# yoshihikoueno/DNNCancerAnnotator

Measured on AMD Instinct MI355X. Metric: MRI slices/sec (fwd+bwd) unet 512x512 bs=8, higher is better.
Workload: dtype f32; 1 GPU; configs/unet.yaml train step (fwd + weighted BCE + bwd + Adam), batch 8 x 512x512x1 per GPU, f32, random-init weights; global_batch=8, parallelism=dp1, kernels=tuned, communicator=False

## Files before the change

### dnncancerannotator_amd/csrc/debug_tools.hip

```cpp
#include "fast.h"
#include "kernels.h"
#include "model.h"
#include <vector>

using namespace dnnca;

typedef float dbg_f32x4 __attribute__((ext_vector_type(4)));
template <int MODE, int NCH>
__global__ __launch_bounds__(512) void k_mfma_rate(float* out, int iters) {
    __shared__ float lds[16384];
    for (int i = threadIdx.x; i < 16384; i += 512) lds[i] = (float)(i & 7) * 0.125f;
    __syncthreads();
    const int lane = threadIdx.x & 63, wave = threadIdx.x >> 6;
    dbg_f32x4 acc[NCH];
    for (int c = 0; c < NCH; ++c) acc[c] = dbg_f32x4{0.f, 0.f, 0.f, 0.f};
    float a = 1.0f + lane * 0.001f, b = 0.5f;
    const int base = wave * 1024 + (lane & 15) * 12 + (lane >> 4);
    for (int it = 0; it < iters; ++it) {
#pragma unroll
        for (int k = 0; k < 16; ++k)
#pragma unroll
            for (int c = 0; c < NCH; ++c) {
                float av = MODE >= 1 ? lds[base + c * 200 + 4 * k + (it & 1) * 64] : a;
                float bv = MODE == 2 ? lds[8192 + base + 4 * k + (it & 1) * 64] : b;
// ... 41 lines not shown
int dnnca_debug_bn_table(void* model, double* abs_sum, unsigned* ticket_sum, int* allocated) {
    MODEL(model);
    *abs_sum = 0.0;
    *ticket_sum = 0u;
    *allocated = M->bn_tab != nullptr;
    if (!M->bn_tab) return DNNCA_OK;
    HIP_TRY(hipStreamSynchronize(M->stream));
    std::vector<double> h(Model::kBnTab + 32);
    HIP_TRY(hipMemcpy(h.data(), M->bn_tab, h.size() * 8, hipMemcpyDeviceToHost));
    for (int i = 0; i < Model::kBnTab; ++i) *abs_sum += h[i] < 0 ? -h[i] : h[i];
    const unsigned* t = reinterpret_cast<const unsigned*>(h.data() + Model::kBnTab);
    for (int i = 0; i < 64; ++i) *ticket_sum += t[i];
    return DNNCA_OK;
}

int dnnca_debug_tcf_dgrads(void* model, int batch, float* dskip, size_t n_skip, float* dtcin, size_t n_tcin) {
    MODEL(model);
    for (size_t i = M->ops.size(); i-- > 1;) {
        const Op& o = M->ops[i];
        const Op& tc = M->ops[i - 1];
        if (o.type != OP_CONV || !o.inB.d.C || o.inA.d.C != 3 || o.inB.d.C != 3 || o.out.d.C != 3) continue;
        if (tc.type != OP_TCONV || tc.inA.d.C != 6 || tc.out.d.p != o.inA.d.p) continue;
        const size_t ns = (size_t)batch * o.out.d.H * o.out.d.W * 3, nt = (size_t)batch * tc.inA.d.H * tc.inA.d.W * 6;
        if (ns != n_skip || nt != n_tcin || !o.inB.g.p || !tc.inA.g.p) { set_error("dnnca_debug_tcf_dgrads: sizes %zu / %zu expected", ns, nt); return DNNCA_EINVAL; }
        HIP_TRY(hipStreamSynchronize(M->stream));
        HIP_TRY(hipMemcpy(dskip, o.inB.g.p, ns * 4, hipMemcpyDeviceToHost));
        HIP_TRY(hipMemcpy(dtcin, tc.inA.g.p, nt * 4, hipMemcpyDeviceToHost));
        return DNNCA_OK;
    }
    set_error("dnnca_debug_tcf_dgrads: no two-source 3-channel conv behind a 6 -> 3 transposed conv");
    return DNNCA_EINVAL;
}

int dnnca_debug_join(void* model, int what, int B, int H, int W, int C, int ps, int c0, int grid, int generic, const float* in0,
                     const float* in1, float* io0, float* io1, const float* coef, double* sums, int acc0, int acc1) {
    MODEL(model);
    if (what < 0 || what > 2 || B < 1 || H < 1 || W < 1 || C < 1 || c0 < 0 || c0 + C > ps || !in0 || !in1 || !io0 || (what == 2 && !io1) ||
        (what == 1 && !coef) || (generic && what == 1)) { set_error("dnnca_debug_join: bad arguments"); return DNNCA_EINVAL; }
    const size_t n = (size_t)B * H * W * ps;
    float* dev = nullptr;
    const size_t n4 = (n + 3) / 4 * 4;
    double* dsum = nullptr;
    unsigned* ticket = nullptr;
    float* dcoef = nullptr;
    const unsigned rows = (unsigned)(grid > 0 ? grid : 0) + (unsigned)((C + 255) / 256);
    const size_t part = std::max(join_part_doubles(C), (size_t)rows * C);
    hipStream_t s = M->stream;
    int rc = DNNCA_OK;
    auto body = [&]() -> int {
        HIP_TRY(hipMalloc(&dev, 4 * n4 * 4));
        HIP_TRY(hipMalloc(&dsum, (2 * (size_t)C + part) * 8));
        HIP_TRY(hipMalloc(&ticket, 16));
        HIP_TRY(hipMalloc(&dcoef, 2 * (size_t)C * 4));
        HIP_TRY(hipMemsetAsync(ticket, 0, 16, s));
        HIP_TRY(hipMemsetAsync(dsum, 0xff, (2 * (size_t)C + part) * 8, s));
        HIP_TRY(hipMemcpyAsync(dev, in0, n * 4, hipMemcpyHostToDevice, s));
        HIP_TRY(hipMemcpyAsync(dev + n4, in1, n * 4, hipMemcpyHostToDevice, s));
        HIP_TRY(hipMemcpyAsync(dev + 2 * n4, io0, n * 4, hipMemcpyHostToDevice, s));
        if (io1) HIP_TRY(hipMemcpyAsync(dev + 3 * n4, io1, n * 4, hipMemcpyHostToDevice, s));
        if (coef) HIP_TRY(hipMemcpyAsync(dcoef, coef, 2 * (size_t)C * 4, hipMemcpyHostToDevice, s));
        View v[4];
        for (int k = 0; k < 4; ++k) { v[k].p = dev + k * n4 + c0; v[k].H = H; v[k].W = W; v[k].C = C; v[k].ps = ps; }
        if (what == 0) {
            if (generic) g_join_fwd(s, B, v[0], v[1], v[2]);
            else join_fwd(s, B, v[0], v[1], v[2], sums ? dsum : nullptr, dsum + 2 * C, ticket, grid);
        } else if (what == 1) {
// ... 26 lines not shown
```

### dnncancerannotator_amd/csrc/fz_dev.h

```cpp
#pragma once
#include <hip/hip_runtime.h>

namespace dnnca {
namespace fz {

typedef float f32x4 __attribute__((ext_vector_type(4)));

constexpr int cdiv(int a, int b) { return (a + b - 1) / b; }
constexpr int up4(int a) { return (a + 3) / 4 * 4; }

template <int C, int G, int RG, int ROWS, int HALO>
struct Tile {
    static constexpr int LEAD = (4 - (HALO * C) % 4) % 4;
    static constexpr int LS = RG * G * C;
    static constexpr int LS4 = LS / 4;
    static_assert(LS % 4 == 0, "tile rows must be whole float4's");
    static constexpr int N = up4(LEAD + (ROWS + 2) * LS + 20 * G * C + 16);
    static constexpr int N4 = N / 4;
};

__device__ __forceinline__ void lds_barrier() { asm volatile("s_waitcnt lgkmcnt(0)\n\ts_barrier" ::: "memory"); }
__device__ __forceinline__ float act(float v, float alpha) { return alpha < 0.f ? v : (v > 0.f ? v : alpha * v); }


template <int C, int G, int RG, int ROWS, int HALO, int WPX, int LSF, int NT>
struct Stager {
    static constexpr int LEAD = (4 - (HALO * C) % 4) % 4;
    static constexpr int W4 = (LEAD + WPX * C + 3) / 4;
    static constexpr int LS4 = LSF / 4;
    static_assert(W4 <= LS4 && LSF % 4 == 0, "tile row narrower than the staged width");
    static constexpr int NPF = cdiv(ROWS * W4, NT);
    float4 pre[NPF];
    unsigned ok;
    __device__ __forceinline__ void issue(const float* __restrict__ src, int b, int y0, int x0, int H, int W, int tid) {
        const int rowlen4 = W * C / 4;
        const int f40 = ((x0 - HALO) * C - LEAD) / 4;
        const float4* base = reinterpret_cast<const float4*>(src) + (size_t)b * H * rowlen4;
        const int last = H * rowlen4 - 1;
        ok = 0;
#pragma unroll
        for (int k = 0; k < NPF; ++k) {
            const int idx = tid + k * NT;
            const int r = idx / W4, c4 = idx - r * W4;
            const int gy = y0 - HALO + r, g4 = f40 + c4;
            ok |= (idx < ROWS * W4 && (unsigned)gy < (unsigned)H && (unsigned)g4 < (unsigned)rowlen4) ? (1u << k) : 0u;
            pre[k] = base[min(max(gy * rowlen4 + g4, 0), last)];
        }
    }
    __device__ __forceinline__ void commit(float* lds, int tid) const {
#pragma unroll
        for (int k = 0; k < NPF; ++k) {
            const int idx = tid + k * NT;
            const int r = idx / W4, c4 = idx - r * W4;
            if (idx < ROWS * W4) reinterpret_cast<float4*>(lds)[r * LS4 + c4] = (ok >> k) & 1u ? pre[k] : make_float4(0.f, 0.f, 0.f, 0.f);
        }
    }
};

template <int C, int G, int RG, int ROWS, int HALO, int TW, int TH, int NT>
__device__ __forceinline__ void store_interior(const float* lds, float* __restrict__ dst, int b, int y0, int x0, int H, int W, int tid) {
    using TL = Tile<C, G, RG, ROWS, HALO>;
    constexpr int R4 = TW * C / 4;
    constexpr int OFF = TL::LEAD + HALO * C;
    static_assert(OFF % 4 == 0 && (TW * C) % 4 == 0, "unaligned tile interior");
    float* base = dst + ((size_t)b * H + y0) * W * C + (size_t)x0 * C;
    for (int idx = tid; idx < TH * R4; idx += NT) {
        const int r = idx / R4, c4 = idx - r * R4;
        const float4 v = *reinterpret_cast<const float4*>(lds + (HALO + r) * TL::LS + OFF + 4 * c4);
        *reinterpret_cast<float4*>(base + (size_t)r * W * C + 4 * c4) = v;
    }
}

template <int C, int G, int RG, int OROWS, int OW, int LEAD, int NT>
__device__ __forceinline__ void zero_ring(float* t, unsigned edge, int tid) {
    constexpr int LS = RG * G * C;
    if (edge & 1u) for (int i = tid; i < OW * C; i += NT) t[LEAD + i] = 0.f;
    if (edge & 2u) for (int i = tid; i < OW * C; i += NT) t[LEAD + (OROWS - 1) * LS + i] = 0.f;
    if (edge & 4u) for (int i = tid; i < OROWS * C; i += NT) t[LEAD + (i / C) * LS + (i % C)] = 0.f;
    if (edge & 8u) for (int i = tid; i < OROWS * C; i += NT) t[LEAD + (i / C) * LS + (OW - 1) * C + (i % C)] = 0.f;
}

template <int C, int NSRC, int CO, int RG, int OROWS, int ILEAD, int ISTRIDE, int OLEAD, int NW, int MPR>
struct Conv3 {
    static constexpr int G = 12 / CO, GC = G * C, WR = (G + 2) * C, SR = (WR + 3) / 4, KS = NSRC * 3 * SR, ILS = RG * GC;
    static constexpr int NMT = MPR ? OROWS * MPR : cdiv(OROWS * RG, 16), CH = cdiv(NMT, NW);
    static_assert(MPR == 0 || (NW % MPR == 0 && NMT % NW == 0), "row-aligned M-tiles must divide evenly over the waves");
    static constexpr int CSTEP = MPR ? (NW / MPR) * RG * GC : NW * 16 * GC;
// ... 71 lines not shown
```

### dnncancerannotator_amd/csrc/kernels_fused_bwd.hip

```cpp
#include <stdio.h>
#include <stdlib.h>
#include <string.h>
#include <type_traits>

#include "fast.h"
#include "fz_dev.h"
#include "kernels.h"

namespace dnnca {
namespace fzb {

using namespace fz;

template <int C, int CO, int RG, int OROWS, int ILEAD, int OLEAD, int NW, int MPR>
struct DConv3 {
    static constexpr int G = 12 / CO, GC = G * C, WR = (G + 2) * C, SR = (WR + 3) / 4, KS = 3 * SR, ILS = RG * GC;
    static constexpr int NMT = MPR ? OROWS * MPR : cdiv(OROWS * RG, 16), CH = cdiv(NMT, NW);
    static_assert(MPR == 0 || (NW % MPR == 0 && NMT % NW == 0), "row-aligned M-tiles must divide evenly over the waves");
    static constexpr int CSTEP = MPR ? RG * GC : NW * 16 * GC;

    static __device__ __forceinline__ void run(const float* in, float* out, const float* breg, const float* msk, float malpha, int wave, int lane) {
        const int m = lane & 15, q = lane >> 4, n = m;
        constexpr bool RAGGED = CH * NW > NMT;
        const bool last_ok = !RAGGED || wave + (CH - 1) * NW < NMT;
// ... 100 lines not shown
    do {                                                                                                              \
        if (lane == 0 && (wave == 0 || wave == NWD) && blockIdx.x < 1024 && (i) < 32) g_fzb_stamps[((KID * 1024 + blockIdx.x) * 2 + (role)) * 32 + (i)] = fzb_now(); \
    } while (0)
#else
#define FZB_STAMP(role, i) do { } while (0)
#endif

struct BArgs {
    const float* dz1;
    const float* y1;
    const float* dpool;
    const unsigned char* pidx;
    float pf_alpha;
    const float* y0;
    const float* xa;
    const float* xb;
    const float* bm1;
    const float* bm0;
    float* dxb;
    int mask0;
    float alpha0;
    float* slabs1;
    float* slabs0[2];
    const float* tc_in;
    float* tc_din;
    const float* tc_w;
    float* tc_slabs;
    int tc_mask;
    float tc_alpha;
    int B, H, W, tiles_x, tiles_y;
    int dbg;
};

template <bool UP, int CA, int F, int TW, int NT, int ISSUE_DG = 2, int ISSUE_WG = 2>
__global__ __launch_bounds__(NT, 1) void k_fzb(BArgs p) {
    constexpr int TH = 8, NW = NT / 64, NWD = NW / 2, NWW = NW - NWD, NSRC = UP ? 2 : 1, CT = 12;
    constexpr int KID = (UP ? 0 : 2) + (F == 12 ? 1 : 0);
    (void)KID;
    static_assert(!UP || CA == F, "decoder block: both sources of the first conv have F channels");
    constexpr int G = 12 / F, RG = even_up(cdiv(TW + 5, G)), PR = RG * G;
    using TDZ1 = Tile<F, G, RG, TH + 4, 2>;
    using TY0 = Tile<F, G, RG, TH + 2, 1>;
    using TXA = Tile<CA, G, RG, TH + 2, 1>;
    constexpr int CO2 = UP ? 12 : CA, G2 = 12 / CO2, NPASS = UP ? (2 * F) / 12 : 1, RG2I = PR / G2, MPR2 = (TW / G2) / 16, OUT2 = TH * TW * CO2;
    static_assert(PR % G2 == 0 && (TW / G2) % 16 == 0, "second-stage groups must tile the rows");
    using DC1 = DConv3<F, F, RG, TH + 2, TDZ1::LEAD, TY0::LEAD, NWD, 0>;
    using DC0 = DConv3<F, CO2, RG2I, TH, TY0::LEAD, 0, NWD, MPR2>;
    using W1 = WG<F, F, TW>;
    using W0 = WG<CA, F, TW>;
    using SDZ = Stager<F, G, RG, TH + 4, 2, TW + 4, TDZ1::LS, NT>;
    using SY0 = Stager<F, G, RG, TH + 2, 1, TW + 2, TY0::LS, NT>;
    using SXA = Stager<CA, G, RG, TH + 2, 1, TW + 2, TXA::LS, NT>;
    constexpr int LWt = TW / 2, NLP = (TH / 2) * LWt, KA = 2 * F, KS1t = KA / 4, KTt = 4 * F, MBt = cdiv(KTt, 16), ROWF = TW * 12;
    using SLO = Stager<CT, 1, 1, TH / 2, 0, TW / 2, LWt * CT, NT>;
    static_assert(!UP || (LWt % 16 == 0 && KA % 4 == 0), "UP: whole M-tiles per low-resolution row");
    constexpr int PFR = TH / 2 + 2, PFW = TW / 2 + 2, PFLEAD = (4 - F % 4) % 4, PFLS = up4(PFLEAD + PFW * F), PFLI = PFLS / 4, PFN4 = PFR * PFLI;
    constexpr int NPS = UP ? 1 : cdiv(PFN4, NT);
    constexpr int O_DZ1 = 0, O_Y0 = O_DZ1 + TDZ1::N, O_DZ0 = O_Y0 + TY0::N, O_XA = O_DZ0 + TY0::N, O_EXT = O_XA + NSRC * TXA::N;
    constexpr int O_LOW = O_EXT, O_TCW = O_LOW + NLP * CT;
    constexpr int O_PDP = O_EXT, O_PIX = O_PDP + PFN4 * 4;
    constexpr int O_CST = UP ? O_TCW + KTt * CT : O_PIX + PFN4, O_ROW = O_CST + 4;
    constexpr int O_BM1 = O_ROW + NWD * 192, O_BM0 = O_BM1 + DC1::KS * 64, LDSN = O_BM0 + NPASS * DC0::KS * 64;
    constexpr int O_OUT = O_DZ1;
    static_assert(NPASS * OUT2 <= TDZ1::N, "stage-2 output tiles must fit the dz1 tile");
    constexpr int MT1 = W1::MT, MT0 = W0::MT;
    constexpr int ACCF = (MT1 + NSRC * MT0) * 256;
    constexpr int TACCF = UP ? MBt * 256 : 0;
    static_assert(NWW * ACCF + NWD * TACCF <= LDSN, "the final reduction must fit the LDS");
    constexpr int RPW = TH / (NWD / MPR2), LPW = 8 * (RPW / 2);
    static_assert(NWD % MPR2 == 0 && TH % (NWD / MPR2) == 0 && (!UP || (RPW % 2 == 0 && LPW % 16 == 0)), "wave rectangles");
    static_assert(LDSN * 4 <= 160 * 1024, "LDS budget");
    __shared__ float4 lds4[(LDSN + 3) / 4];
    float* lds = reinterpret_cast<float*>(lds4);
    const float* ldsf = lds;
    constexpr int CST1 = O_CST, CST0 = O_CST + 1;

    const int tid = threadIdx.x, lane = tid & 63;
    const int wave = __builtin_amdgcn_readfirstlane(tid >> 6);
    const int ntiles = p.tiles_x * p.tiles_y * p.B;
#ifdef DNNCA_TUNING
    const bool xcd_map = (ntiles & 7) == 0 && (gridDim.x & 7) == 0 && !(p.dbg & 4);
#else
    const bool xcd_map = (ntiles & 7) == 0 && (gridDim.x & 7) == 0;
#endif

    SDZ sdz;
    SY0 sy0;
    SXA sxa[NSRC];
    SDZ sy1;
    SLO slo;
    float4 predp[NPS];
    unsigned preix[NPS];
    auto issue = [&](int b, int x0, int y0) {
        sdz.issue(p.dz1, b, y0, x0, p.H, p.W, tid);
        if constexpr (!UP) {
            sy1.issue(p.y1, b, y0, x0, p.H, p.W, tid);
            const int Hp = p.H >> 1, Wp = p.W >> 1, rowf = Wp * F;
#pragma unroll
            for (int k = 0; k < NPS; ++k) {
                const int id = tid + k * NT;
                const int r = id / PFLI, c4 = id - r * PFLI;
                const int gy = (y0 >> 1) - 1 + r, gf = ((x0 >> 1) - 1) * F - PFLEAD + 4 * c4;
                const bool ok = id < PFN4 && (unsigned)gy < (unsigned)Hp && gf >= 0 && gf < rowf;
                const size_t off = ok ? ((size_t)b * Hp + gy) * rowf + gf : 0;
                predp[k] = *reinterpret_cast<const float4*>(p.dpool + off);
                if (!ok) predp[k] = make_float4(0.f, 0.f, 0.f, 0.f);
                preix[k] = *reinterpret_cast<const unsigned*>(p.pidx + off);
                if (!ok) preix[k] = 0xffffffffu;
            }
        }
        sy0.issue(p.y0, b, y0, x0, p.H, p.W, tid);
        sxa[0].issue(p.xa, b, y0, x0, p.H, p.W, tid);
        if constexpr (UP) {
            sxa[1].issue(p.xb, b, y0, x0, p.H, p.W, tid);
            slo.issue(p.tc_in, b, y0 >> 1, x0 >> 1, p.H >> 1, p.W >> 1, tid);
        }
    };
    auto commit = [&]() {
        if constexpr (!UP) {
#pragma unroll
            for (int k = 0; k < NPS; ++k) {
                const int id = tid + k * NT;
                if (id < PFN4) {
                    reinterpret_cast<float4*>(lds + O_PDP)[id] = predp[k];
                    reinterpret_cast<unsigned*>(lds + O_PIX)[id] = preix[k];
                }
            }
            lds_barrier();
            const unsigned char* ixb = reinterpret_cast<const unsigned char*>(lds + O_PIX);
            const float* pdp = lds + O_PDP;
            static_assert(SDZ::LEAD == 0 && F % 2 == 0 && PFLS % 2 == 0 && (PFLEAD % 2) == 0, "PF transform works on aligned channel pairs");
#pragma unroll
            for (int k = 0; k < SDZ::NPF; ++k) {
                const int idx = tid + k * NT;
                const int r = idx / SDZ::W4, c4 = idx - r * SDZ::W4;
                float g[4] = {sdz.pre[k].x, sdz.pre[k].y, sdz.pre[k].z, sdz.pre[k].w};
                const float yv[4] = {sy1.pre[k].x, sy1.pre[k].y, sy1.pre[k].z, sy1.pre[k].w};
                const int f0 = 4 * c4;
                if (((sdz.ok >> k) & 1u) && f0 < (TW + 4) * F) {
                    const int px0 = f0 / F, ch0 = f0 - px0 * F;
                    const int pr = ((r - 2) >> 1) + 1;
                    const unsigned rowbit = ((unsigned)r & 1u) << 1;
#pragma unroll
                    for (int h = 0; h < 2; ++h) {
                        int ch = ch0 + 2 * h, px = px0;
                        if (ch >= F) { ch -= F; ++px; }
                        const int pc = ((px - 2) >> 1) + 1;
                        const unsigned pos = rowbit | ((unsigned)px & 1u);
                        const int o = pr * PFLS + PFLEAD + pc * F + ch;
                        const float2 dp = *reinterpret_cast<const float2*>(pdp + o);
                        const unsigned ix = *reinterpret_cast<const unsigned short*>(ixb + o);
                        g[2 * h] = (g[2 * h] + ((ix & 0xffu) == pos ? dp.x : 0.f)) * (yv[2 * h] > 0.f ? 1.0f : p.pf_alpha);
                        g[2 * h + 1] = (g[2 * h + 1] + ((ix >> 8) == pos ? dp.y : 0.f)) * (yv[2 * h + 1] > 0.f ? 1.0f : p.pf_alpha);
                    }
                }
                sdz.pre[k] = make_float4(g[0], g[1], g[2], g[3]);
            }
        }
        sdz.commit(lds + O_DZ1, tid);
        sy0.commit(lds + O_Y0, tid);
        sxa[0].commit(lds + O_XA, tid);
        if constexpr (UP) {
            sxa[1].commit(lds + O_XA + TXA::N, tid);
            slo.commit(lds + O_LOW, tid);
        }
    };

    FZB_STAMP(wave >= NWD, 0);
    int tile = blockIdx.x;
    int b = 0, x0 = 0, y0 = 0;
    if (tile < ntiles) {
        decode_tile(tile, ntiles, xcd_map, p.tiles_x, p.tiles_y, TW, TH, b, x0, y0);
        issue(b, x0, y0);
    }
#ifdef DNNCA_TUNING
    if (p.dbg & 8) {
        FZB_STAMP(wave >= NWD, 25);
        asm volatile("s_waitcnt vmcnt(0)" ::: "memory");
        FZB_STAMP(wave >= NWD, 26);
    }
#endif
    constexpr int KSA = DC1::KS + NPASS * DC0::KS, NBR = cdiv(KSA, NW);
    static_assert(O_BM0 == O_BM1 + DC1::KS * 64, "bm1 and bm0 adjacent in LDS");
    float pbm[NBR];
#pragma unroll
    for (int k = 0; k < NBR; ++k) {
        const int s = min(wave + k * NW, KSA - 1);
        pbm[k] = s < DC1::KS ? p.bm1[s * 64 + lane] : p.bm0[(s - DC1::KS) * 64 + lane];
    }
    constexpr int NTW = UP ? cdiv(KTt * CT, NT) : 1;
    float ptw[NTW];
    if constexpr (UP) {
#pragma unroll
        for (int k = 0; k < NTW; ++k) ptw[k] = p.tc_w[min(tid + k * NT, KTt * CT - 1)];
    }
    FZB_STAMP(wave >= NWD, 27);
    for (int i = tid; i < (LDSN + 3) / 4; i += NT) lds4[i] = make_float4(0.f, 0.f, 0.f, 0.f);
    FZB_STAMP(wave >= NWD, 28);
    __syncthreads();
    FZB_STAMP(wave >= NWD, 29);
    if (tid == 0) lds[CST1] = 1.0f;
#pragma unroll
    for (int k = 0; k < NBR; ++k)
        if (wave + k * NW < KSA) lds[O_BM1 + (wave + k * NW) * 64 + lane] = pbm[k];
    if constexpr (UP) {
#pragma unroll
        for (int k = 0; k < NTW; ++k)
            if (tid + k * NT < KTt * CT) lds[O_TCW + tid + k * NT] = ptw[k];
    }
    if (tile >= ntiles) return;

    int cb = b, cx0 = x0, cy0 = y0;
    FZB_STAMP(wave >= NWD, 1);
    commit();
    tile += gridDim.x;
    lds_barrier();
    FZB_STAMP(wave >= NWD, 2);

    auto role = [&](auto tag) {
        constexpr bool DG = decltype(tag)::value;
        const int wv = DG ? wave : wave - NWD;
        f32x4 acc1[1][MT1], acc0[NSRC][MT0], tacc[UP ? MBt : 1];
        W1 w1;
        W0 w0;
        if constexpr (DG) {
#pragma unroll
            for (int t = 0; t < (UP ? MBt : 1); ++t) tacc[t] = f32x4{0.f, 0.f, 0.f, 0.f};
        }
        if constexpr (!DG) {
#pragma unroll
            for (int t = 0; t < MT1; ++t) acc1[0][t] = f32x4{0.f, 0.f, 0.f, 0.f};
#pragma unroll
            for (int s = 0; s < NSRC; ++s)
#pragma unroll
                for (int t = 0; t < MT0; ++t) acc0[s][t] = f32x4{0.f, 0.f, 0.f, 0.f};
            w1.init(lane, TY0::LEAD, TY0::LS, CST1, CST0);
            w0.init(lane, TXA::LEAD, TXA::LS, CST1, CST0);
        }
        int it = 0;
        (void)it;
#pragma unroll 1
        for (;; ++it) {
            const unsigned edge = tile_edge(cx0, cy0, TW, TH, p.H, p.W);
            FZB_STAMP(!DG, it < 3 ? 3 + 8 * it : 99);
            auto prefetch = [&]() {
                decode_tile(tile < ntiles ? tile : tile - (int)gridDim.x, ntiles, xcd_map, p.tiles_x, p.tiles_y, TW, TH, b, x0, y0);
                issue(b, x0, y0);
            };
            constexpr int ISSUE_AT = DG ? ISSUE_DG : ISSUE_WG;
            if constexpr (ISSUE_AT == 1) prefetch();
            __builtin_amdgcn_s_setprio(DG ? 2 : 0);
            if constexpr (DG) {
                float breg[DC1::KS];
                load_breg<DC1::KS>(breg, lds + O_BM1, lane);
                DC1::run(lds + O_DZ1, lds + O_DZ0, breg, p.mask0 ? lds + O_Y0 : nullptr, p.alpha0, wv, lane);
            } else {
#pragma unroll 1
                for (int ty = wv; ty < TH; ty += NWW) {
                    const int xr[1] = {O_Y0 + ty * TY0::LS};
                    w1.template row<1>(acc1, ldsf, xr, O_DZ1 + TDZ1::LEAD + (ty + 2) * TDZ1::LS + 2 * F, CST0, lane);
                }
            }
            FZB_STAMP(!DG, it < 3 ? 4 + 8 * it : 99);
            lds_barrier();
            FZB_STAMP(!DG, it < 3 ? 5 + 8 * it : 99);
            if (edge && !(p.mask0 && p.alpha0 == 0.f)) {
                zero_ring<F, G, RG, TH + 2, TW + 2, TY0::LEAD, NT>(lds + O_DZ0, edge, tid);
                lds_barrier();
            }
            __builtin_amdgcn_s_setprio(0);
            if constexpr (ISSUE_AT == 2) prefetch();
            if constexpr (DG) {
#pragma unroll
                for (int ps = 0; ps < NPASS; ++ps) {
                    float breg[DC0::KS];
                    load_breg<DC0::KS>(breg, lds + O_BM0 + ps * DC0::KS * 64, lane);
                    DC0::run(lds + O_DZ0, lds + O_OUT + ps * OUT2, breg, nullptr, 0.f, wv, lane);
                }
                __builtin_amdgcn_wave_barrier();
                const int r0 = (wv / MPR2) * RPW, cbk = wv % MPR2;
                if constexpr (UP) {
                    float* base = p.dxb + ((size_t)cb * p.H + cy0 + r0) * p.W * F + (size_t)(cx0 + cbk * 16) * F;
                    if constexpr (NPASS == 2) {
                        static_assert(F == 12, "two passes: 12 channels per pass");
                        if (lane < 48) {
#pragma unroll
                            for (int rr = 0; rr < RPW; ++rr)
                                *reinterpret_cast<float4*>(base + (size_t)rr * p.W * F + 4 * lane) =
                                    *reinterpret_cast<const float4*>(lds + O_OUT + OUT2 + (r0 + rr) * ROWF + cbk * 192 + 4 * lane);
                        }
                    } else {
                        static_assert(F == 6, "one pass: [up | skip] of 6 channels each");
                        if (lane < 48) {
                            const int px = (2 * lane) / F, ch = 2 * lane - px * F;
#pragma unroll
                            for (int rr = 0; rr < RPW; ++rr)
                                *reinterpret_cast<float2*>(base + (size_t)rr * p.W * F + 2 * lane) =
                                    *reinterpret_cast<const float2*>(lds + O_OUT + (r0 + rr) * ROWF + (cbk * 16 + px) * 12 + F + ch);
                        }
                    }
                    const int m16 = lane & 15, q = lane >> 4;
                    const int lr0 = r0 / 2, lc0 = cbk * 8;
                    int koff[KS1t];
#pragma unroll
                    for (int kk = 0; kk < KS1t; ++kk) {
                        const int k = 4 * kk + q, e = k / F;
                        koff[kk] = e * 12 + (k - e * F);
                    }
                    const int woff = m16 < CT ? O_TCW + q * CT + m16 : CST0, wstep = m16 < CT ? 4 * CT : 0;
                    float* orow = lds + O_ROW + wv * 192;
#pragma unroll
// ... 52 lines not shown
#pragma unroll
                        for (int t = 0; t < MBt; ++t) tav[i][t] = ldsf[offT[t] + (valT[t] ? sd : 0)];
                    }
                    __builtin_amdgcn_sched_barrier(0);
#pragma unroll
                    for (int i = 0; i < KST; ++i)
#pragma unroll
                        for (int t = 0; t < MBt; ++t) tacc[t] = __builtin_amdgcn_mfma_f32_16x16x4f32(tav[i][t], tbv[i], tacc[t], 0, 0, 0);
                } else {
                    static_assert(MPR2 == 1 && TW * CA == 192, "DOWN: a wave stores whole rows of 48 float4");
                    float* base = p.dxb + ((size_t)cb * p.H + cy0 + r0) * p.W * CA + (size_t)cx0 * CA;
                    if (lane < 48) {
#pragma unroll
                        for (int rr = 0; rr < RPW; ++rr)
                            *reinterpret_cast<float4*>(base + (size_t)rr * p.W * CA + 4 * lane) =
                                *reinterpret_cast<const float4*>(lds + O_OUT + (r0 + rr) * (TW * CA) + 4 * lane);
                    }
                }
            } else {
#pragma unroll 1
                for (int ty = wv; ty < TH; ty += NWW) {
                    int xr[NSRC];
#pragma unroll
                    for (int s = 0; s < NSRC; ++s) xr[s] = O_XA + s * TXA::N + ty * TXA::LS;
                    w0.template row<NSRC>(acc0, ldsf, xr, O_DZ0 + TY0::LEAD + (ty + 1) * TY0::LS + F, CST0, lane);
                }
            }
            FZB_STAMP(!DG, it < 3 ? 8 + 8 * it : 99);
            const bool more = tile < ntiles;
            if (!more) break;
            lds_barrier();
            FZB_STAMP(!DG, it < 3 ? 9 + 8 * it : 99);
            cb = b; cx0 = x0; cy0 = y0;
            commit();
            tile += gridDim.x;
            if constexpr (DG) __builtin_amdgcn_s_waitcnt(0x0070);
            lds_barrier();
            FZB_STAMP(!DG, it < 3 ? 10 + 8 * it : 99);
        }
        lds_barrier();
        if constexpr (!DG) {
            float* red = lds + wv * ACCF;
#pragma unroll
            for (int t = 0; t < MT1; ++t)
#pragma unroll
                for (int r = 0; r < 4; ++r) red[(t * 4 + r) * 64 + lane] = acc1[0][t][r];
#pragma unroll
            for (int s = 0; s < NSRC; ++s)
#pragma unroll
                for (int t = 0; t < MT0; ++t)
#pragma unroll
                    for (int r = 0; r < 4; ++r) red[(MT1 + s * MT0 + t) * 256 + r * 64 + lane] = acc0[s][t][r];
        } else if constexpr (UP) {
            float* red = lds + NWW * ACCF + wv * TACCF;
#pragma unroll
            for (int t = 0; t < MBt; ++t)
#pragma unroll
                for (int r = 0; r < 4; ++r) red[t * 256 + r * 64 + lane] = tacc[t][r];
        }
    };
    if (wave < NWD) role(std::true_type{});
    else role(std::false_type{});
    __syncthreads();
    FZB_STAMP(wave >= NWD, 30);
#ifdef DNNCA_TUNING
    if (p.dbg & 1) return;
#endif
    const int bucket = blockIdx.x % kPgBuckets;
    auto flush = [&](int first, int nw, int stride, int mt, float* slab, int rows, int cols) {
        for (int i = tid; i < mt * 256; i += NT) {
            const int t = i >> 8, r = (i >> 6) & 3, ln = i & 63;
            if ((ln & 15) < cols && 16 * t + 4 * (ln >> 4) + r < rows) {
                float v = 0.f;
                for (int w = 0; w < nw; ++w) v += lds[first + w * stride + i];
                atomicAdd(slab + (size_t)bucket * (mt * 256) + i, v);
            }
        }
    };
    flush(0, NWW, ACCF, MT1, p.slabs1, W1::MROWS, 12);
#pragma unroll
    for (int s = 0; s < NSRC; ++s) flush((MT1 + s * MT0) * 256, NWW, ACCF, MT0, p.slabs0[s], W0::MROWS, 12);
    if constexpr (UP) flush(NWW * ACCF, NWD, TACCF, MBt, p.tc_slabs, KTt, CT + 1);
    FZB_STAMP(wave >= NWD, 31);
}

}


constexpr int kFzbPerCu = 2;

static bool fzb_selected(const Model* m, const char* kind, int F) {
    return m->sw.fzb_only.empty() || m->sw.fzb_only == kind + std::to_string(F == 6 ? 1 : 2);
}

bool fused_up_bwd(Model* m, int B, size_t oi) {
    if (m->sw.no_fused_bwd || (m->desc.flags & 1) || m->desc.dtype != DNNCA_F32 || oi < 2 || oi >= m->ops.size()) return false;
    Op &tc = m->ops[oi - 2], &c0 = m->ops[oi - 1], &c1 = m->ops[oi];
    if (tc.type != OP_TCONV || c0.type != OP_CONV || c1.type != OP_CONV || tc.k != 2 || c0.k != 3 || c1.k != 3) return false;
    if (!fast_pg_conv_supported(m, c0) || !fast_pg_conv_supported(m, c1) || !fast_tconv_supported(m, tc)) return false;
    if (c0.inA.d.p != tc.out.d.p || !c0.inB.d.C || c1.inB.d.C || c1.inA.d.p != c0.out.d.p) return false;
    const int F = c1.out.d.C, H = c1.out.d.H, W = c1.out.d.W;
    if (!(F == 6 || F == 12) || tc.inA.d.C != 12 || tc.out.d.C != F || c0.inA.d.C != F || c0.inB.d.C != F || c0.out.d.C != F || c1.inA.d.C != F) return false;
    if (tc.inA.d.H * 2 != H || tc.inA.d.W * 2 != W || c0.out.d.H != H || c0.out.d.W != W || c0.inB.d.H != H || c0.inB.d.W != W) return false;
    const int TW = 32 * (12 / F);
    if (W % TW || H % 8) return false;
    if (!dense(tc.inA.d) || !dense(tc.inA.g) || !dense(tc.out.d) || !dense(c0.inB.d) || !dense(c0.inB.g) || !dense(c0.out.d) || !dense(c1.out.g)) return false;
    if (c1.alpha >= 0.f && !c1.premasked) return false;
    if (!c1.need_din || !c0.need_din || c1.accA || c0.accA || c0.accB || c0.maskA || c0.maskB || tc.accA) return false;
    if ((c0.alpha >= 0.f) != (c1.maskA != 0) || (c0.alpha >= 0.f && !c0.premasked)) return false;
    if (!fzb_selected(m, "up", F)) return false;
    fzb::BArgs a{};
    a.dz1 = c1.out.g.p;
    a.y0 = c0.out.d.p;
    a.xa = c0.inA.d.p; a.xb = c0.inB.d.p;
    a.bm1 = fast_conv_bmat_dgrad(m, c1); a.bm0 = fast_conv_bmat_dgrad(m, c0);
    a.dxb = c0.inB.g.p;
    a.mask0 = c1.maskA; a.alpha0 = c1.mask_alpha;
    a.slabs1 = fast_wgrad_slabs(m, c1, 0);
    a.slabs0[0] = fast_wgrad_slabs(m, c0, 0); a.slabs0[1] = fast_wgrad_slabs(m, c0, 1);
    a.tc_in = tc.inA.d.p; a.tc_din = tc.inA.g.p; a.tc_w = m->p + tc.w_off; a.tc_slabs = fast_wgrad_slabs(m, tc, 0);
    a.tc_mask = tc.maskA; a.tc_alpha = tc.mask_alpha;
    if (!a.bm1 || !a.bm0 || !a.slabs1 || !a.slabs0[0] || !a.slabs0[1] || !a.tc_slabs) return false;
    a.B = B; a.H = H; a.W = W;
    a.tiles_x = W / TW; a.tiles_y = H / 8;
    a.dbg = m->sw.fzb_dbg;
    const int ntiles = a.tiles_x * a.tiles_y * B;
    const double npx = (double)B * H * W;
    const double bytes = 4.0 * npx * ((F + 2 * F) + (F + 2 * 2 * F) + 2 * (F + 0.25 * 12));
    const double flops = 2.0 * (2.0 * npx * 9.0 * (F * F + 2 * F * F)) + 2.0 * (2.0 * npx * F * 12);
#define X(f, tw)                                                                                                   \
    if (F == f) {                                                                                                  \
        const int g = resident_grid<fzb::k_fzb<true, f, f, tw, 512>, 512>(kFzbPerCu, ntiles);                      \
        if (a.dbg & 2) {         \
            fzb::BArgs a2 = a;                                                                                     \
            a2.dbg |= 1;                                                                                           \
            LAUNCH(m, "fzb_up_pre_" #f, bytes, flops,                                                              \
                   hipLaunchKernelGGL((fzb::k_fzb<true, f, f, tw, 512>), dim3(g), dim3(512), 0, m->stream, a2));   \
        }                                                                                                          \
        LAUNCH(m, "fzb_up_" #f, bytes, flops,                                                                      \
               hipLaunchKernelGGL((fzb::k_fzb<true, f, f, tw, 512>), dim3(g), dim3(512), 0, m->stream, a));        \
        return true;                                                                                               \
    }
    X(12, 32) X(6, 64)
#undef X
    return false;
}

bool fused_down_bwd(Model* m, int B, size_t oi) {
    if (m->sw.no_fused_bwd || (m->desc.flags & 1) || m->desc.dtype != DNNCA_F32 || oi < 2 || oi >= m->ops.size()) return false;
    Op &c1 = m->ops[oi - 2], &c2 = m->ops[oi - 1], &pl = m->ops[oi];
    if (c1.type != OP_CONV || c2.type != OP_CONV || pl.type != OP_POOL || c1.k != 3 || c2.k != 3 || pl.k != 2) return false;
    if (!fast_pg_conv_supported(m, c1) || !fast_pg_conv_supported(m, c2)) return false;
    if (c1.inB.d.C || c2.inB.d.C || c2.inA.d.p != c1.out.d.p || pl.inA.d.p != c2.out.d.p) return false;
    const int CA = c1.inA.d.C, F = c1.out.d.C, H = c1.out.d.H, W = c1.out.d.W;
    if (!((CA == 6 && F == 12) || (CA == 3 && F == 6)) || c2.out.d.C != F) return false;
    const int TW = 32 * (12 / F);
    if (W % TW || H % 8) return false;
    if (!dense(c1.inA.d) || !dense(c1.inA.g) || !dense(c1.out.d) || !dense(c2.out.d) || !dense(c2.out.g) || !dense(pl.out.g) || !dense(pl.out.d)) return false;
    if (!pl.pool_idx_valid || !(pl.pool_idx || m->dry) || !pl.accA || !pl.maskA || pl.mask_alpha != 0.f || !c2.premasked) return false;
    if (!c1.need_din || !c2.need_din || c1.accA || c1.maskA || c2.accA) return false;
    if ((c1.alpha >= 0.f) != (c2.maskA != 0) || (c1.alpha >= 0.f && !c1.premasked)) return false;
    if (!fzb_selected(m, "down", F)) return false;
    fzb::BArgs a{};
    a.dz1 = c2.out.g.p;
    a.y1 = c2.out.d.p;
    a.dpool = pl.out.g.p; a.pidx = pl.pool_idx; a.pf_alpha = pl.mask_alpha;
    a.y0 = c1.out.d.p;
    a.xa = c1.inA.d.p;
    a.bm1 = fast_conv_bmat_dgrad(m, c2); a.bm0 = fast_conv_bmat_dgrad(m, c1);
    a.dxb = c1.inA.g.p;
    a.mask0 = c2.maskA; a.alpha0 = c2.mask_alpha;
    a.slabs1 = fast_wgrad_slabs(m, c2, 0);
    a.slabs0[0] = fast_wgrad_slabs(m, c1, 0);
    if (!a.bm1 || !a.bm0 || !a.slabs1 || !a.slabs0[0]) return false;
    a.B = B; a.H = H; a.W = W;
    a.tiles_x = W / TW; a.tiles_y = H / 8;
    a.dbg = m->sw.fzb_dbg;
    const int ntiles = a.tiles_x * a.tiles_y * B;
    const double npx = (double)B * H * W;
    const double bytes = 4.0 * npx * ((2 * F + 0.5 * F) + (F + 2 * F) + (F + 2 * CA));
    const double flops = 2.0 * (2.0 * npx * 9.0 * (F * F + CA * F));
    pl.pool_idx_valid = false;
#define X(ca, f, tw)                                                                                               \
    if (CA == ca && F == f) {                                                                                      \
        const int g = resident_grid<fzb::k_fzb<false, ca, f, tw, 512>, 512>(kFzbPerCu, ntiles);                    \
        LAUNCH(m, "fzb_down_" #ca "_" #f, bytes, flops,                                                            \
               hipLaunchKernelGGL((fzb::k_fzb<false, ca, f, tw, 512>), dim3(g), dim3(512), 0, m->stream, a));      \
        return true;                                                                                               \
    }
    X(6, 12, 32) X(3, 6, 64)
#undef X
    return false;
}

}

extern "C" int dnnca_debug_fzb_stamps(unsigned long long* out, int n) {
#ifdef DNNCA_TUNING
    if (hipDeviceSynchronize() != hipSuccess) return -1;
    return hipMemcpyFromSymbol(out, HIP_SYMBOL(dnnca::fzb::g_fzb_stamps), (size_t)n * 8) == hipSuccess ? 0 : -1;
#else
    (void)out; (void)n;
    return -2;
#endif
}
```

### dnncancerannotator_amd/csrc/model.h

```cpp
#pragma once
#include <initializer_list>
#include <map>
#include <string>
#include <vector>

#include "common.h"
#include "kernels.h"

typedef struct ncclComm* ncclComm_t;

namespace dnnca {

struct T {
    View d, g;
};

inline T tslice(const T& t, int c0, int c) { return T{slice(t.d, c0, c), slice(t.g, c0, c)}; }

enum OpType { OP_CONV = 0, OP_BN, OP_POOL, OP_TCONV, OP_HEAD, OP_JOIN };

struct Op {
    OpType type;
    std::string name;
    T inA, inB, out;
// ... 21 lines not shown
};

struct ParamInfo {
    std::string name;
    int64_t shape[4];
    int ndim;
    int trainable;
    int64_t offset;
    int64_t size;
};

struct KStat {
    std::string name;
    int64_t launches = 0;
    double total_ms = 0, bytes = 0, flops = 0;
};

constexpr float kBnMomentum = 0.99f;
constexpr float kBnEps = 1e-3f;

struct RegionState;

struct ConfThresholds {
    float* dev = nullptr;
    std::vector<int> order;
    int n = 0;
};

struct StepSwitches {
    bool no_fused = false, no_fused_bwd = false, no_first3 = false, no_first3f = false, no_up3f = false, no_tail3 = false;
    bool no_tcf = false, no_tcm = false, no_tconv_ride = false, no_prep_ride = false, no_fold_adam = false, no_pool_fold = false;
    bool no_bwd3v = false, no_vw = false, no_head_in_conv = false, no_label_fusion = false, no_wg_stream = false;
    bool pgbwd_old = false;
    bool fz_up2 = false, fz_all = false, lockstep = false, force_rccl = false;
    std::string fz_only, fzb_only;
    int stamp_c = 0, stamp_ns = 0, stamp_co = 0;
    bool stamps_pf = false;
    int dbg = 0, fzb_dbg = 0, f3f_abl = 0, abl = 0, tail3_variant = 0;
    int nblocks = 0, pg_maxocc = 3;
    int tail3_slots = 2048, tail3_lds = 0;
    int lockstep_maxh = 128;
    int wg_prio = 1;
    size_t bucket_bytes = 8u << 20;
    bool no_join = false;
};
StepSwitches step_switches();

struct Model {
    dnnca_model_desc desc;
    StepSwitches sw;
    int device = 0;
    hipStream_t stream = nullptr;
    std::vector<ParamInfo> params;
    std::vector<Op> ops;
    std::vector<void*> allocs;
    int64_t nT = 0, nS = 0;
    float *p = nullptr, *g = nullptr, *m = nullptr, *v = nullptr, *state = nullptr;
    double* scalars = nullptr;
    float* out5 = nullptr;
    float *x_stage = nullptr, *y_stage = nullptr, *logits = nullptr, *dlogits = nullptr, *prob = nullptr;
    struct HeadPending { const float* partials = nullptr; int nblocks = 0, C = 0; float* dw = nullptr; float* dbias = nullptr; } head_pending;
    bool head_defer_ok = false;
    bool step_init_done = false;
    struct FinalizePending { bool on = false; dnnca_loss_cfg cfg; double n_label = 0, inv_batch_hw = 0; } fin_pending;
    float* y_smooth = nullptr;
    void* warp_scratch = nullptr;
// ... 165 lines not shown
```

### dnncancerannotator_amd/csrc/model.hip

```cpp
#include "model.h"

#include <rccl/rccl.h>
#include <stdarg.h>
#include <string.h>

#include <algorithm>
#include <cmath>

#include "calib.h"
#include "fast.h"
#include "kernels.h"
#include "region.h"
#include "sens.h"
#include "attr.h"

namespace dnnca {

static thread_local char g_err[1024] = "";

void set_error(const char* fmt, ...) {
    va_list ap;
    va_start(ap, fmt);
    vsnprintf(g_err, sizeof(g_err), fmt, ap);
    va_end(ap);
}

enum { kScalars = 8 };

StepSwitches step_switches() {
    auto on = [](const char* name) { return getenv(name) != nullptr; };
    auto num = [](const char* name, int dflt) { return getenv(name) ? atoi(getenv(name)) : dflt; };
    auto str = [](const char* name) { return std::string(getenv(name) ? getenv(name) : ""); };
    StepSwitches s;
    s.no_fused = on("DNNCA_NO_FUSED");
    s.no_fused_bwd = on("DNNCA_NO_FUSED_BWD");
    s.no_first3 = on("DNNCA_NO_FIRST3");
    s.no_first3f = on("DNNCA_NO_FIRST3F");
    s.no_up3f = on("DNNCA_NO_UP3F");
    s.no_tail3 = on("DNNCA_NO_TAIL3");
    s.no_tcf = on("DNNCA_NO_TCF");
    s.no_tcm = on("DNNCA_NO_TCM");
    s.no_tconv_ride = on("DNNCA_NO_TCONV_RIDE");
    s.no_prep_ride = on("DNNCA_NO_PREP_RIDE");
    s.no_fold_adam = on("DNNCA_NO_FOLD_ADAM");
    s.no_pool_fold = on("DNNCA_NO_POOL_FOLD");
    s.no_bwd3v = on("DNNCA_NO_BWD3V");
    s.no_vw = on("DNNCA_NO_VW");
    s.no_head_in_conv = on("DNNCA_NO_HEAD_IN_CONV");
    s.no_label_fusion = on("DNNCA_NO_LABEL_FUSION");
    s.no_wg_stream = on("DNNCA_NO_WG_STREAM");
    s.pgbwd_old = on("DNNCA_PGBWD_OLD");
    s.fz_up2 = on("DNNCA_FZ_UP2");
    s.fz_all = on("DNNCA_FZ_ALL");
    s.lockstep = on("DNNCA_LOCKSTEP");
    s.force_rccl = on("DNNCA_FORCE_RCCL");
    s.no_join = on("DNNCA_NO_JOIN");
    s.fz_only = str("DNNCA_FZ_ONLY");
    s.fzb_only = str("DNNCA_FZB_ONLY");
    if (sscanf(str("DNNCA_STAMPS").c_str(), "%d,%d,%d", &s.stamp_c, &s.stamp_ns, &s.stamp_co) != 3) s.stamp_c = s.stamp_ns = s.stamp_co = 0;
    s.stamps_pf = on("DNNCA_STAMPS_PF");
    s.dbg = num("DNNCA_DBG", 0);
    s.fzb_dbg = num("DNNCA_FZB_DBG", 0);
    s.f3f_abl = num("DNNCA_F3F_ABL", 0);
    s.abl = num("DNNCA_ABL", 0);
    s.tail3_variant = num("DNNCA_TAIL3_VARIANT", 0);
    s.nblocks = std::max(num("DNNCA_NBLOCKS", 0), 0);
    s.pg_maxocc = num("DNNCA_PG_MAXOCC", 3);
    s.tail3_slots = num("DNNCA_TAIL3_SLOTS", 2048);
    s.tail3_lds = num("DNNCA_TAIL3_LDS", 0);
    s.lockstep_maxh = num("DNNCA_LOCKSTEP_MAXH", 128);
    s.wg_prio = num("DNNCA_WG_PRIO", 1);
    if (const char* e = getenv("DNNCA_BUCKET_BYTES")) s.bucket_bytes = std::max((size_t)atol(e), (size_t)4096);
    return s;
}

static bool head_in_conv_requested(const Model* M, const dnnca_loss_cfg& cfg) {
    return !cfg.label_smoothing && M->merged_launches() && !M->sw.no_head_in_conv;
}

Model::~Model() {
    region_release(this);
    fast_release(this);
    ig_release(this);
    for (void* a : allocs) (void)hipFree(a);
// ... 2734 lines not shown
```

Baseline: 20020 slices/s.

## Split fused upsample backward staging so each role streams its own operands

Adds an SC variant of the fused up-block backward kernel. Only dz and y0 are prefetched across tiles; xa, xb, tc_in and the second-pass weights are now issued by one wave role during phase 1 and committed before the phase-2 barrier. The prologue barrier becomes a partial waitcnt so the bm0 and tc weight loads stay in flight, and y0 is committed inside phase 2. The intent is to cut register-held prefetch state and the stall at the start of each tile, at the cost of more loads on the critical path inside each iteration and more complex synchronisation. An env switch keeps the old path, a debug hook exports block dgrads, and an optional block-count override is added.

```diff
diff --git a/dnncancerannotator_amd/csrc/debug_tools.hip b/dnncancerannotator_amd/csrc/debug_tools.hip
--- a/dnncancerannotator_amd/csrc/debug_tools.hip
+++ b/dnncancerannotator_amd/csrc/debug_tools.hip
@@ -97,6 +97,35 @@
     return DNNCA_EINVAL;
 }
 
+int dnnca_debug_fzb_dgrads(void* model, int batch, int up, int F, float* dxb, size_t n_dxb, float* dtcin, size_t n_tcin) {
+    MODEL(model);
+    for (size_t i = M->ops.size(); i-- > 2;) {
+        const Op& c0 = up ? M->ops[i - 1] : M->ops[i - 2];
+        const float* gx = nullptr;
+        const float* gt = nullptr;
+        size_t nx = 0, nt = 0;
+        if (up) {
+            const Op& tc = M->ops[i - 2];
+            if (c0.type != OP_CONV || c0.inA.d.C != F || c0.inB.d.C != F || c0.out.d.C != F) continue;
+            if (tc.type != OP_TCONV || tc.inA.d.C != 12 || tc.out.d.p != c0.inA.d.p) continue;
+            gx = c0.inB.g.p; nx = (size_t)batch * c0.out.d.H * c0.out.d.W * F;
+            gt = tc.inA.g.p; nt = (size_t)batch * tc.inA.d.H * tc.inA.d.W * 12;
+        } else {
+            const Op& c1 = M->ops[i - 1];
+            if (M->ops[i].type != OP_POOL || c1.type != OP_CONV || c0.type != OP_CONV || c0.inB.d.C || c0.out.d.C != F || c1.out.d.C != F) continue;
+            if (c1.inA.d.p != c0.out.d.p || M->ops[i].inA.d.p != c1.out.d.p) continue;
+            gx = c0.inA.g.p; nx = (size_t)batch * c0.out.d.H * c0.out.d.W * c0.inA.d.C;
+        }
+        if (nx != n_dxb || nt != n_tcin || !gx || (up && !gt)) { set_error("dnnca_debug_fzb_dgrads: sizes %zu / %zu expected", nx, nt); return DNNCA_EINVAL; }
+        HIP_TRY(hipStreamSynchronize(M->stream));
+        HIP_TRY(hipMemcpy(dxb, gx, nx * 4, hipMemcpyDeviceToHost));
+        if (up) HIP_TRY(hipMemcpy(dtcin, gt, nt * 4, hipMemcpyDeviceToHost));
+        return DNNCA_OK;
+    }
+    set_error("dnnca_debug_fzb_dgrads: no %s block of %d channels", up ? "Upsample" : "Downsample", F);
+    return DNNCA_EINVAL;
+}
+
 int dnnca_debug_join(void* model, int what, int B, int H, int W, int C, int ps, int c0, int grid, int generic, const float* in0,
                      const float* in1, float* io0, float* io1, const float* coef, double* sums, int acc0, int acc1) {
     MODEL(model);
diff --git a/dnncancerannotator_amd/csrc/fz_dev.h b/dnncancerannotator_amd/csrc/fz_dev.h
--- a/dnncancerannotator_amd/csrc/fz_dev.h
+++ b/dnncancerannotator_amd/csrc/fz_dev.h
@@ -53,6 +53,15 @@
             const int idx = tid + k * NT;
             const int r = idx / W4, c4 = idx - r * W4;
             if (idx < ROWS * W4) reinterpret_cast<float4*>(lds)[r * LS4 + c4] = (ok >> k) & 1u ? pre[k] : make_float4(0.f, 0.f, 0.f, 0.f);
+        }
+    }
+    __device__ __forceinline__ void commit_all(float* lds, int tid) const {
+        static_assert((NPF * NT - 1) / W4 <= ROWS + 1, "slots past the tile must land in its padding rows");
+#pragma unroll
+        for (int k = 0; k < NPF; ++k) {
+            const int idx = tid + k * NT;
+            const int r = idx / W4, c4 = idx - r * W4;
+            reinterpret_cast<float4*>(lds)[r * LS4 + c4] = (ok >> k) & 1u ? pre[k] : make_float4(0.f, 0.f, 0.f, 0.f);
         }
     }
 };
diff --git a/dnncancerannotator_amd/csrc/kernels_fused_bwd.hip b/dnncancerannotator_amd/csrc/kernels_fused_bwd.hip
--- a/dnncancerannotator_amd/csrc/kernels_fused_bwd.hip
+++ b/dnncancerannotator_amd/csrc/kernels_fused_bwd.hip
@@ -156,7 +156,7 @@
     int dbg;
 };
 
-template <bool UP, int CA, int F, int TW, int NT, int ISSUE_DG = 2, int ISSUE_WG = 2>
+template <bool UP, int CA, int F, int TW, int NT, bool SC = true, int ISSUE_DG = 2, int ISSUE_WG = 2>
 __global__ __launch_bounds__(NT, 1) void k_fzb(BArgs p) {
     constexpr int TH = 8, NW = NT / 64, NWD = NW / 2, NWW = NW - NWD, NSRC = UP ? 2 : 1, CT = 12;
     constexpr int KID = (UP ? 0 : 2) + (F == 12 ? 1 : 0);
@@ -177,6 +177,11 @@
     using SXA = Stager<CA, G, RG, TH + 2, 1, TW + 2, TXA::LS, NT>;
     constexpr int LWt = TW / 2, NLP = (TH / 2) * LWt, KA = 2 * F, KS1t = KA / 4, KTt = 4 * F, MBt = cdiv(KTt, 16), ROWF = TW * 12;
     using SLO = Stager<CT, 1, 1, TH / 2, 0, TW / 2, LWt * CT, NT>;
+    constexpr int NTR = NT / 2;
+    static_assert(NW % 2 == 0, "role-local stagers: both roles have NT / 2 threads");
+    using SY0R = Stager<F, G, RG, TH + 2, 1, TW + 2, TY0::LS, NTR>;
+    using SXAR = Stager<CA, G, RG, TH + 2, 1, TW + 2, TXA::LS, NTR>;
+    using SLOR = Stager<CT, 1, 1, TH / 2, 0, TW / 2, LWt * CT, NTR>;
     static_assert(!UP || (LWt % 16 == 0 && KA % 4 == 0), "UP: whole M-tiles per low-resolution row");
     constexpr int PFR = TH / 2 + 2, PFW = TW / 2 + 2, PFLEAD = (4 - F % 4) % 4, PFLS = up4(PFLEAD + PFW * F), PFLI = PFLS / 4, PFN4 = PFR * PFLI;
     constexpr int NPS = UP ? 1 : cdiv(PFN4, NT);
@@ -215,7 +220,7 @@
     SLO slo;
     float4 predp[NPS];
     unsigned preix[NPS];
-    auto issue = [&](int b, int x0, int y0) {
+    auto issue_dz = [&](int b, int x0, int y0) {
         sdz.issue(p.dz1, b, y0, x0, p.H, p.W, tid);
         if constexpr (!UP) {
             sy1.issue(p.y1, b, y0, x0, p.H, p.W, tid);
@@ -233,6 +238,9 @@
                 if (!ok) preix[k] = 0xffffffffu;
             }
         }
+    };
+    auto issue = [&](int b, int x0, int y0) {
+        issue_dz(b, x0, y0);
         sy0.issue(p.y0, b, y0, x0, p.H, p.W, tid);
         sxa[0].issue(p.xa, b, y0, x0, p.H, p.W, tid);
         if constexpr (UP) {
@@ -240,7 +248,7 @@
             slo.issue(p.tc_in, b, y0 >> 1, x0 >> 1, p.H >> 1, p.W >> 1, tid);
         }
     };
-    auto commit = [&]() {
+    auto commit_dz = [&]() {
         if constexpr (!UP) {
 #pragma unroll
             for (int k = 0; k < NPS; ++k) {
@@ -282,6 +290,9 @@
             }
         }
         sdz.commit(lds + O_DZ1, tid);
+    };
+    auto commit = [&]() {
+        commit_dz();
         sy0.commit(lds + O_Y0, tid);
         sxa[0].commit(lds + O_XA, tid);
         if constexpr (UP) {
@@ -293,7 +304,11 @@
     FZB_STAMP(wave >= NWD, 0);
     int tile = blockIdx.x;
     int b = 0, x0 = 0, y0 = 0;
-    if (tile < ntiles) {
+    if constexpr (SC) {
+        decode_tile(min(tile, ntiles - 1), ntiles, xcd_map, p.tiles_x, p.tiles_y, TW, TH, b, x0, y0);
+        issue_dz(b, x0, y0);
+        sy0.issue(p.y0, b, y0, x0, p.H, p.W, tid);
+    } else if (tile < ntiles) {
         decode_tile(tile, ntiles, xcd_map, p.tiles_x, p.tiles_y, TW, TH, b, x0, y0);
         issue(b, x0, y0);
     }
@@ -306,11 +321,19 @@
 #endif
     constexpr int KSA = DC1::KS + NPASS * DC0::KS, NBR = cdiv(KSA, NW);
     static_assert(O_BM0 == O_BM1 + DC1::KS * 64, "bm1 and bm0 adjacent in LDS");
-    float pbm[NBR];
-#pragma unroll
-    for (int k = 0; k < NBR; ++k) {
-        const int s = min(wave + k * NW, KSA - 1);
+    constexpr int KSB = SC ? DC1::KS : KSA, NBR1 = cdiv(KSB, NW), KS0A = KSA - DC1::KS, NBR0 = SC ? cdiv(KS0A, NW) : 1;
+    (void)NBR;
+    float pbm[NBR1], pbm0[NBR0];
+    if constexpr (SC) __builtin_amdgcn_sched_barrier(0);
+#pragma unroll
+    for (int k = 0; k < NBR1; ++k) {
+        const int s = min(wave + k * NW, KSB - 1);
         pbm[k] = s < DC1::KS ? p.bm1[s * 64 + lane] : p.bm0[(s - DC1::KS) * 64 + lane];
+    }
+    if constexpr (SC) {
+        __builtin_amdgcn_sched_barrier(0);
+#pragma unroll
+        for (int k = 0; k < NBR0; ++k) pbm0[k] = p.bm0[min(wave + k * NW, KS0A - 1) * 64 + lane];
     }
     constexpr int NTW = UP ? cdiv(KTt * CT, NT) : 1;
     float ptw[NTW];
@@ -318,16 +341,33 @@
 #pragma unroll
         for (int k = 0; k < NTW; ++k) ptw[k] = p.tc_w[min(tid + k * NT, KTt * CT - 1)];
     }
+    auto commit_p2_operands = [&]() {
+#pragma unroll
+        for (int k = 0; k < NBR0; ++k)
+            if (wave + k * NW < KS0A) lds[O_BM0 + (wave + k * NW) * 64 + lane] = pbm0[k];
+        if constexpr (UP) {
+#pragma unroll
+            for (int k = 0; k < NTW; ++k)
+                if (tid + k * NT < KTt * CT) lds[O_TCW + tid + k * NT] = ptw[k];
+        }
+    };
     FZB_STAMP(wave >= NWD, 27);
     for (int i = tid; i < (LDSN + 3) / 4; i += NT) lds4[i] = make_float4(0.f, 0.f, 0.f, 0.f);
     FZB_STAMP(wave >= NWD, 28);
-    __syncthreads();
+    if constexpr (SC) {
+        lds_barrier();
+        constexpr int YOUNGER = NBR0 + (UP ? NTW : 0);
+        static_assert(YOUNGER < 64, "vmcnt has six bits");
+        __builtin_amdgcn_s_waitcnt((YOUNGER & 15) | ((YOUNGER >> 4) << 14) | 0x0f70);
+    } else {
+        __syncthreads();
+    }
     FZB_STAMP(wave >= NWD, 29);
     if (tid == 0) lds[CST1] = 1.0f;
 #pragma unroll
-    for (int k = 0; k < NBR; ++k)
-        if (wave + k * NW < KSA) lds[O_BM1 + (wave + k * NW) * 64 + lane] = pbm[k];
-    if constexpr (UP) {
+    for (int k = 0; k < NBR1; ++k)
+        if (wave + k * NW < KSB) lds[O_BM1 + (wave + k * NW) * 64 + lane] = pbm[k];
+    if constexpr (!SC && UP) {
 #pragma unroll
         for (int k = 0; k < NTW; ++k)
             if (tid + k * NT < KTt * CT) lds[O_TCW + tid + k * NT] = ptw[k];
@@ -336,7 +376,12 @@
 
     int cb = b, cx0 = x0, cy0 = y0;
     FZB_STAMP(wave >= NWD, 1);
-    commit();
+    if constexpr (SC) {
+        commit_dz();
+        sy0.commit(lds + O_Y0, tid);
+    } else {
+        commit();
+    }
     tile += gridDim.x;
     lds_barrier();
     FZB_STAMP(wave >= NWD, 2);
@@ -344,6 +389,12 @@
     auto role = [&](auto tag) {
         constexpr bool DG = decltype(tag)::value;
         const int wv = DG ? wave : wave - NWD;
+        constexpr bool ST_XA = SC && (DG == (F == 12)), ST_XB = SC && UP && DG;
+        const int rt = DG ? tid : tid - NWD * 64;
+        SY0R sy0r;
+        SXAR sxar[NSRC];
+        SLOR slor;
+        (void)rt; (void)sy0r; (void)sxar; (void)slor;
         f32x4 acc1[1][MT1], acc0[NSRC][MT0], tacc[UP ? MBt : 1];
         W1 w1;
         W0 w0;
@@ -369,10 +420,21 @@
             FZB_STAMP(!DG, it < 3 ? 3 + 8 * it : 99);
             auto prefetch = [&]() {
                 decode_tile(tile < ntiles ? tile : tile - (int)gridDim.x, ntiles, xcd_map, p.tiles_x, p.tiles_y, TW, TH, b, x0, y0);
-                issue(b, x0, y0);
+                if constexpr (SC) {
+                    if constexpr (DG) sy0r.issue(p.y0, b, y0, x0, p.H, p.W, rt);
+                    issue_dz(b, x0, y0);
+                } else {
+                    issue(b, x0, y0);
+                }
             };
             constexpr int ISSUE_AT = DG ? ISSUE_DG : ISSUE_WG;
+            static_assert(!SC || (ISSUE_DG == 2 && ISSUE_WG == 2), "SC: y0 is prefetched and committed inside P2");
             if constexpr (ISSUE_AT == 1) prefetch();
+            if constexpr (ST_XA) sxar[0].issue(p.xa, cb, cy0, cx0, p.H, p.W, rt);
+            if constexpr (ST_XB) {
+                sxar[1].issue(p.xb, cb, cy0, cx0, p.H, p.W, rt);
+                slor.issue(p.tc_in, cb, cy0 >> 1, cx0 >> 1, p.H >> 1, p.W >> 1, rt);
+            }
             __builtin_amdgcn_s_setprio(DG ? 2 : 0);
             if constexpr (DG) {
                 float breg[DC1::KS];
@@ -385,6 +447,14 @@
                     w1.template row<1>(acc1, ldsf, xr, O_DZ1 + TDZ1::LEAD + (ty + 2) * TDZ1::LS + 2 * F, CST0, lane);
                 }
             }
+            if constexpr (SC) {
+                if constexpr (ST_XA) sxar[0].commit(lds + O_XA, rt);
+                if constexpr (ST_XB) {
+                    sxar[1].commit(lds + O_XA + TXA::N, rt);
+                    slor.commit(lds + O_LOW, rt);
+                }
+                commit_p2_operands();
+            }
             FZB_STAMP(!DG, it < 3 ? 4 + 8 * it : 99);
             lds_barrier();
             FZB_STAMP(!DG, it < 3 ? 5 + 8 * it : 99);
@@ -401,6 +471,7 @@
                     load_breg<DC0::KS>(breg, lds + O_BM0 + ps * DC0::KS * 64, lane);
                     DC0::run(lds + O_DZ0, lds + O_OUT + ps * OUT2, breg, nullptr, 0.f, wv, lane);
                 }
+                if constexpr (SC) sy0r.commit_all(lds + O_Y0, rt);
                 __builtin_amdgcn_wave_barrier();
                 const int r0 = (wv / MPR2) * RPW, cbk = wv % MPR2;
                 if constexpr (UP) {
@@ -519,7 +590,8 @@
             lds_barrier();
             FZB_STAMP(!DG, it < 3 ? 9 + 8 * it : 99);
             cb = b; cx0 = x0; cy0 = y0;
-            commit();
+            if constexpr (SC) commit_dz();
+            else commit();
             tile += gridDim.x;
             if constexpr (DG) __builtin_amdgcn_s_waitcnt(0x0070);
             lds_barrier();
@@ -575,6 +647,12 @@
 
 
 constexpr int kFzbPerCu = 2;
+
+template <auto Kernel>
+static int fzb_grid(const Model* m, int ntiles) {
+    const int g = resident_grid<Kernel, 512>(kFzbPerCu, ntiles);
+    return m->sw.nblocks > 0 ? std::max(1, std::min(m->sw.nblocks, g)) : g;
+}
 
 static bool fzb_selected(const Model* m, const char* kind, int F) {
     return m->sw.fzb_only.empty() || m->sw.fzb_only == kind + std::to_string(F == 6 ? 1 : 2);
@@ -615,20 +693,20 @@
     const double npx = (double)B * H * W;
     const double bytes = 4.0 * npx * ((F + 2 * F) + (F + 2 * 2 * F) + 2 * (F + 0.25 * 12));
     const double flops = 2.0 * (2.0 * npx * 9.0 * (F * F + 2 * F * F)) + 2.0 * (2.0 * npx * F * 12);
-#define X(f, tw)                                                                                                   \
-    if (F == f) {                                                                                                  \
-        const int g = resident_grid<fzb::k_fzb<true, f, f, tw, 512>, 512>(kFzbPerCu, ntiles);                      \
+#define X(f, tw, sc)                                                                                               \
+    if (F == f && m->sw.fzb_old == !sc) {                                                                          \
+        const int g = fzb_grid<fzb::k_fzb<true, f, f, tw, 512, sc>>(m, ntiles);                                    \
         if (a.dbg & 2) {         \
             fzb::BArgs a2 = a;                                                                                     \
             a2.dbg |= 1;                                                                                           \
             LAUNCH(m, "fzb_up_pre_" #f, bytes, flops,                                                              \
-                   hipLaunchKernelGGL((fzb::k_fzb<true, f, f, tw, 512>), dim3(g), dim3(512), 0, m->stream, a2));   \
+                   hipLaunchKernelGGL((fzb::k_fzb<true, f, f, tw, 512, sc>), dim3(g), dim3(512), 0, m->stream, a2)); \
         }                                                                                                          \
         LAUNCH(m, "fzb_up_" #f, bytes, flops,                                                                      \
-               hipLaunchKernelGGL((fzb::k_fzb<true, f, f, tw, 512>), dim3(g), dim3(512), 0, m->stream, a));        \
+               hipLaunchKernelGGL((fzb::k_fzb<true, f, f, tw, 512, sc>), dim3(g), dim3(512), 0, m->stream, a));    \
         return true;                                                                                               \
     }
-    X(12, 32) X(6, 64)
+    X(12, 32, true) X(6, 64, true) X(12, 32, false) X(6, 64, false)
 #undef X
     return false;
 }
@@ -670,9 +748,9 @@
     pl.pool_idx_valid = false;
 #define X(ca, f, tw)                                                                                               \
     if (CA == ca && F == f) {                                                                                      \
-        const int g = resident_grid<fzb::k_fzb<false, ca, f, tw, 512>, 512>(kFzbPerCu, ntiles);                    \
+        const int g = fzb_grid<fzb::k_fzb<false, ca, f, tw, 512, false>>(m, ntiles);                               \
         LAUNCH(m, "fzb_down_" #ca "_" #f, bytes, flops,                                                            \
-               hipLaunchKernelGGL((fzb::k_fzb<false, ca, f, tw, 512>), dim3(g), dim3(512), 0, m->stream, a));      \
+               hipLaunchKernelGGL((fzb::k_fzb<false, ca, f, tw, 512, false>), dim3(g), dim3(512), 0, m->stream, a)); \
         return true;                                                                                               \
     }
     X(6, 12, 32) X(3, 6, 64)
diff --git a/dnncancerannotator_amd/csrc/model.h b/dnncancerannotator_amd/csrc/model.h
--- a/dnncancerannotator_amd/csrc/model.h
+++ b/dnncancerannotator_amd/csrc/model.h
@@ -77,6 +77,7 @@
     bool no_tcf = false, no_tcm = false, no_tconv_ride = false, no_prep_ride = false, no_fold_adam = false, no_pool_fold = false;
     bool no_bwd3v = false, no_vw = false, no_head_in_conv = false, no_label_fusion = false, no_wg_stream = false;
     bool pgbwd_old = false;
+    bool fzb_old = false;
     bool fz_up2 = false, fz_all = false, lockstep = false, force_rccl = false;
     std::string fz_only, fzb_only;
     int stamp_c = 0, stamp_ns = 0, stamp_co = 0;
diff --git a/dnncancerannotator_amd/csrc/model.hip b/dnncancerannotator_amd/csrc/model.hip
--- a/dnncancerannotator_amd/csrc/model.hip
+++ b/dnncancerannotator_amd/csrc/model.hip
@@ -50,6 +50,7 @@
     s.no_label_fusion = on("DNNCA_NO_LABEL_FUSION");
     s.no_wg_stream = on("DNNCA_NO_WG_STREAM");
     s.pgbwd_old = on("DNNCA_PGBWD_OLD");
+    s.fzb_old = on("DNNCA_FZB_OLD");
     s.fz_up2 = on("DNNCA_FZ_UP2");
     s.fz_all = on("DNNCA_FZ_ALL");
     s.lockstep = on("DNNCA_LOCKSTEP");
```

New measurement: 20090 slices/s, median of 6. Within noise of the previous version (+0.3%).
